# witalis3/UHSDR

Measured on AMD Instinct MI355X. Metric: Msamples/s through full SSB-RX chain (node); % of HBM-roofline per GPU, higher is better.
Workload: dtype f32; 1 GPU; C2: 4096 ch x 256-frame blocks, SSB-USB P48 chain, f32; channels_per_gpu=4096, frames_per_call=256, parallelism=channel-sharded x1, no data-path collective, outputs=f32 audio, pipelined=True, handoff=persistent, precision=exact, schedule=split_pipe

## Files before the change

### uhsdr_amd/csrc/uhsdr_dsp.h

```cpp
#ifndef UHSDR_DSP_H
#define UHSDR_DSP_H

#include <hip/hip_runtime.h>
#include <stdint.h>
#include "uhsdr_internal.h"

#define BLK UHSDR_IQ_BLOCK_SIZE
#define IQ_BIT_SCALE_DOWN 0.0000152587890625f

typedef float vf4 __attribute__((ext_vector_type(4)));

template <int V, int N>
__device__ __forceinline__ void lds_vec(const float* p, float (&w)[N], int j)
{
    if (V == 4)
    {
        const float4 v = *(const float4*)p;
        w[j] = v.x; w[j + 1] = v.y; w[j + 2] = v.z; w[j + 3] = v.w;
    }
    else
    {
        const float2 v = *(const float2*)p;
        w[j] = v.x; w[j + 1] = v.y;
    }
}

typedef const __attribute__((address_space(4))) float ctaps_t;
__device__ __forceinline__ ctaps_t* as_taps(const float* p) { return (ctaps_t*)p; }

template <bool F, typename V>
__device__ __forceinline__ V fir_mac(V acc, V x, V c)
{
    if constexpr (F) return __builtin_elementwise_fma(x, c, acc);
    else return acc + x * c;
}

template <int T, int R, int M, int V = 4, bool F = false, bool TP = false>
__device__ __forceinline__ void fir_block(const float* win, ctaps_t* c, float (&acc)[R])
{
    constexpr int WA = (M * (R - 1) + 8 + 7) & ~7;
    constexpr int NCH = T / 8, TR = T % 8;
    constexpr int ROT = NCH <= 8 ? (NCH > 0 ? NCH : 1) : WA / 8 + 1;
    float w[WA];
#pragma unroll
    for (int r = 0; r < R; ++r) acc[r] = 0.0f;
#pragma unroll
    for (int j = 0; j < WA; j += V) lds_vec<V>(win + j, w, j);
    float cn[8];
    if constexpr (TP)
    {
#pragma unroll
        for (int q = 0; q < 8; ++q) cn[q] = c[q];
    }
#pragma unroll ROT
    for (int ch = 0; ch < NCH; ++ch)
    {
        float cc[8];
        if constexpr (TP)
        {
#pragma unroll
            for (int q = 0; q < 8; ++q) cc[q] = cn[q];
#pragma unroll
            for (int q = 0; q < 8; ++q) cn[q] = c[8 * (ch + 1) + q];
        }
        else
        {
#pragma unroll
            for (int q = 0; q < 8; ++q) cc[q] = c[8 * ch + q];
        }
        float nw[8];
#pragma unroll
        for (int q = 0; q < 8; q += V) lds_vec<V>(win + 8 * ch + WA + q, nw, q);
#pragma unroll
        for (int kk = 0; kk < 8; ++kk)
        {
#pragma unroll
            for (int r = 0; r < R; ++r) acc[r] = fir_mac<F>(acc[r], w[r * M + kk], cc[kk]);
        }
#pragma unroll
        for (int j = 0; j < WA - 8; ++j) w[j] = w[j + 8];
#pragma unroll
        for (int q = 0; q < 8; ++q) w[WA - 8 + q] = nw[q];
    }
#pragma unroll
    for (int kk = 0; kk < TR; ++kk)
    {
        const float ck = TP ? cn[kk] : c[8 * NCH + kk];
#pragma unroll
        for (int r = 0; r < R; ++r) acc[r] = fir_mac<F>(acc[r], w[r * M + kk], ck);
    }
}

typedef float v2f __attribute__((ext_vector_type(2)));
typedef const __attribute__((address_space(4))) v2f ctaps2_t;
__device__ __forceinline__ ctaps2_t* as_taps2(const float* p) { return (ctaps2_t*)p; }

template <int PB>
__host__ __device__ constexpr int pwin_off(int i) { return 2 * i + PB * (i >> 3); }
__host__ __device__ constexpr int front_pad1(int R, bool decim_first, int M) { return R == 8 && (decim_first || M == 1) ? 4 : 0; }

template <int T, int R, int M, bool F = false, int PB = 0, bool TP = false>
__device__ __forceinline__ void fir_block2(const float* win, ctaps2_t* c, v2f (&acc)[R])
{
    constexpr int WA = (M * (R - 1) + 8 + 7) & ~7;
    constexpr int NCH = T / 8, TR = T % 8;
    constexpr int ROT = WA / 8 + 1;
    v2f w[WA];
#pragma unroll
    for (int r = 0; r < R; ++r) acc[r] = v2f{ 0.0f, 0.0f };
#pragma unroll
    for (int j = 0; j < WA; j += 2)
    {
        const vf4 v = *(const vf4*)(win + pwin_off<PB>(j));
        w[j] = v.xy; w[j + 1] = v.zw;
    }
    v2f cn[8];
    if constexpr (TP)
    {
#pragma unroll
        for (int q = 0; q < 8; ++q) cn[q] = c[q];
    }
#pragma unroll ROT
    for (int ch = 0; ch < NCH; ++ch)
    {
        v2f cc[8];
        if constexpr (TP)
        {
#pragma unroll
            for (int q = 0; q < 8; ++q) cc[q] = cn[q];
#pragma unroll
            for (int q = 0; q < 8; ++q) cn[q] = c[8 * (ch + 1) + q];
        }
        else
        {
#pragma unroll
            for (int q = 0; q < 8; ++q) cc[q] = c[8 * ch + q];
        }
        v2f nw[8];
#pragma unroll
        for (int q = 0; q < 8; q += 2)
        {
            const vf4 v = *(const vf4*)(win + (16 + PB) * ch + pwin_off<PB>(WA + q));
            nw[q] = v.xy; nw[q + 1] = v.zw;
        }
#pragma unroll
        for (int kk = 0; kk < 8; ++kk)
        {
#pragma unroll
            for (int r = 0; r < R; ++r) acc[r] = fir_mac<F>(acc[r], w[r * M + kk], cc[kk]);
        }
#pragma unroll
        for (int j = 0; j < WA - 8; ++j) w[j] = w[j + 8];
#pragma unroll
        for (int q = 0; q < 8; ++q) w[WA - 8 + q] = nw[q];
    }
#pragma unroll
    for (int kk = 0; kk < TR; ++kk)
    {
        const v2f ck = TP ? cn[kk] : c[8 * NCH + kk];
#pragma unroll
        for (int r = 0; r < R; ++r) acc[r] = fir_mac<F>(acc[r], w[r * M + kk], ck);
    }
}

constexpr int FRONT_TAIL = 8;

__device__ __forceinline__ float to_vgpr(float x)
{
    float r;
    asm volatile("v_mov_b32 %0, %1" : "=v"(r) : "s"(x));
    return r;
}
template <int N>
__device__ __forceinline__ void to_vgpr(float (&x)[N])
{
#pragma unroll
// ... 224 lines not shown
        const int q = lane + FRONT_WAVE_L * i;
        buf[i] = h[q < qmax ? q : qmax];
    }
}

template <int T, int PB = 0, int HQM>
__device__ __forceinline__ void group_fill_prow(float* smem, int LW, const float* row, int c0, int cpw, int nlive,
                                                int lane, const vf4 (&buf)[HQM])
{
    constexpr int hp4 = hist_p4(T), HQ = hist_qp(T);
    const int nq = cpw * hp4;
#pragma unroll
    for (int i = 0; i < HQ; ++i)
    {
        const int q = lane + FRONT_WAVE_L * i;
        if (q < nq) *(vf4*)(smem + (q / hp4) * LW + pwin_off<PB>(2 * (q % hp4))) = buf[i];
    }
    const vf4* h = (const vf4*)(row + (size_t)c0 * (hp4 * 4));
    const int qmax = nlive * hp4 - 1;
    for (int q = lane + FRONT_WAVE_L * HQ; q < nq; q += FRONT_WAVE_L)
        *(vf4*)(smem + (q / hp4) * LW + pwin_off<PB>(2 * (q % hp4))) = h[q < qmax ? q : qmax];
}

template <int T, int PB = 0>
__device__ __forceinline__ void group_store_prow(const float* smem, int LW, float* row, int c0, int nlive, int lane, int nnew)
{
    constexpr int hp4 = hist_p4(T);
    vf4* h = (vf4*)(row + (size_t)c0 * (hp4 * 4));
    for (int q = lane; q < nlive * hp4; q += FRONT_WAVE_L)
        h[q] = *(const vf4*)(smem + (q / hp4) * LW + pwin_off<PB>(nnew + 2 * (q % hp4)));
}

template <int PB = 0>
__device__ __forceinline__ void window_new2(float* W, int T, bool act, int b, const v2f* vals, int NV)
{
    if (act)
    {
        const int i0 = T - 1 + b * NV;
        if (((T - 1) & 1) == 0)
            for (int j = 0; j < NV; j += 2)
                *(vf4*)(W + pwin_off<PB>(i0 + j)) = vf4{ vals[j].x, vals[j].y, vals[j + 1].x, vals[j + 1].y };
        else
            for (int j = 0; j < NV; ++j) *(v2f*)(W + pwin_off<PB>(i0 + j)) = vals[j];
    }
}

__device__ __forceinline__ void window_new(float* W, int T, bool act, int b, const float* vals, int NV)
{
    if (act)
    {
        float* d = W + T - 1 + b * NV;
        if (((T - 1 + b * NV) & 3) == 0 && (NV & 3) == 0)
            for (int j = 0; j < NV; j += 4) *(vf4*)(d + j) = vf4{ vals[j], vals[j + 1], vals[j + 2], vals[j + 3] };
        else if (((T - 1 + b * NV) & 1) == 0 && (NV & 1) == 0)
            for (int j = 0; j < NV; j += 2) *(v2f*)(d + j) = v2f{ vals[j], vals[j + 1] };
        else
            for (int j = 0; j < NV; ++j) d[j] = vals[j];
    }
}

__host__ __device__ inline void front_lane(int l, int nb, int S, int& g, int& b)
{
    const int cpw = 64 / nb, K = 64 / S, cpg = S / 4;
    if ((nb & (nb - 1)) || nb < K || cpw < cpg)
    {
        g = l / nb;
        b = l % nb;
        return;
    }
    const int h = l & 31;
    int k, j;
    if (h < 4) { k = 0; j = h; }
    else if (h < 12) { k = 1; j = h - 4; }
    else if (h < 16) { k = 0; j = h - 8; }
    else if (h < 20) { k = 1; j = h - 8; }
    else if (h < 28) { k = 0; j = h - 12; }
    else { k = 1; j = h - 16; }
    k += (l >> 5) * 2;
    const int pr = k * cpg + j / K;
    g = pr % cpw;
    b = (pr / cpw) * K + j % K;
}

template <int S>
__device__ __forceinline__ float lattice_step(float x, float (&g)[S > 0 ? S : 1], const float* k, const float* v)
{
    float fcurr = x, fnext = 0.0f, acc = 0.0f;
    float gn[S > 0 ? S : 1];
#pragma unroll
    for (int i = 0; i < S; ++i)
    {
        const float gcurr = g[i];
        fnext = fcurr - (k[i] * gcurr);
        const float gnext = (fnext * k[i]) + gcurr;
        acc += (gnext * v[i]);
        gn[i] = gnext;
        fcurr = fnext;
    }
    acc += (fnext * v[S]);
#pragma unroll
    for (int i = 0; i + 1 < S; ++i) g[i] = gn[i + 1];
    if (S > 0) g[S - 1] = fnext;
    return acc;
}

template <int S, int PAR>
__device__ __forceinline__ float lattice_step_pk(float x, float (&g)[S > 0 ? S : 1], const float* k, const float* v)
{
    if constexpr (S < 3) return lattice_step<S>(x, g, k, v);
    else
    {
        float gn[S], q[S];
        float f = x;
        int i = 0;
        if (PAR)
        {
            f = f - (k[0] * g[0]);
            gn[0] = (f * k[0]) + g[0];
            q[0] = gn[0] * v[0];
            i = 1;
        }
#pragma unroll
        for (; i + 1 < S; i += 2)
        {
            const v2f gp = v2f{ g[i], g[i + 1] }, kp = v2f{ k[i], k[i + 1] };
            const v2f kg = kp * gp;
            const float f0 = f - kg.x;
            const float f1 = f0 - kg.y;
            const v2f gnp = (v2f{ f0, f1 } * kp) + gp;
            const v2f qp = gnp * v2f{ v[i], v[i + 1] };
            gn[i] = gnp.x; gn[i + 1] = gnp.y;
            q[i] = qp.x; q[i + 1] = qp.y;
            f = f1;
        }
        if (i < S)
        {
            f = f - (k[i] * g[i]);
            gn[i] = (f * k[i]) + g[i];
            q[i] = gn[i] * v[i];
        }
        float acc = 0.0f;
#pragma unroll
        for (int j = 0; j < S; ++j) acc += q[j];
        acc += (f * v[S]);
#pragma unroll
        for (int j = 0; j + 1 < S; ++j) g[j] = gn[j + 1];
        g[S - 1] = f;
        return acc;
    }
}

template <int S>
__device__ __forceinline__ void lattice_step2_pk(float x0, float x1, float (&g)[S > 0 ? S : 1], const float* k,
                                                 const float* v, float& y0, float& y1)
{
    static_assert(S >= 3, "packed form");
    float q[2][S + 1];
#pragma unroll
    for (int h = 0; h < 2; ++h)
    {
        float gn[S];
        float f = h ? x1 : x0;
        int i = 0;
        if (h)
        {
            f = f - (k[0] * g[0]);
            gn[0] = (f * k[0]) + g[0];
            q[h][0] = gn[0] * v[0];
            i = 1;
        }
#pragma unroll
        for (; i + 1 < S; i += 2)
        {
            const v2f gp = v2f{ g[i], g[i + 1] }, kp = v2f{ k[i], k[i + 1] };
            const v2f kg = kp * gp;
            const float f0 = f - kg.x;
            const float f1 = f0 - kg.y;
            const v2f gnp = (v2f{ f0, f1 } * kp) + gp;
            const v2f qp = gnp * v2f{ v[i], v[i + 1] };
            gn[i] = gnp.x; gn[i + 1] = gnp.y;
            q[h][i] = qp.x; q[h][i + 1] = qp.y;
            f = f1;
        }
        if (i < S)
        {
            f = f - (k[i] * g[i]);
            gn[i] = (f * k[i]) + g[i];
            q[h][i] = gn[i] * v[i];
        }
        q[h][S] = f * v[S];
#pragma unroll
        for (int j = 0; j + 1 < S; ++j) g[j] = gn[j + 1];
        g[S - 1] = f;
    }
    v2f acc = v2f{ 0.0f, 0.0f };
#pragma unroll
    for (int j = 0; j <= S; ++j) acc = acc + v2f{ q[0][j], q[1][j] };
    y0 = acc.x;
    y1 = acc.y;
}

__device__ __forceinline__ float biquad_step(float x, float& x1, float& x2, float& y1, float& y2, const float* c)
{
    const float acc = (c[0] * x) + (c[1] * x1) + (c[2] * x2) + (c[3] * y1) + (c[4] * y2);
    x2 = x1; x1 = x; y2 = y1; y1 = acc;
    return acc;
}

enum LdsOp { LDS_R128, LDS_W128, LDS_W64, LDS_W32 };
static const int kB128Groups[4][16] = {
    { 0, 1, 2, 3, 12, 13, 14, 15, 20, 21, 22, 23, 24, 25, 26, 27 },
    { 4, 5, 6, 7, 8, 9, 10, 11, 16, 17, 18, 19, 28, 29, 30, 31 },
    { 32, 33, 34, 35, 44, 45, 46, 47, 52, 53, 54, 55, 56, 57, 58, 59 },
    { 36, 37, 38, 39, 40, 41, 42, 43, 48, 49, 50, 51, 60, 61, 62, 63 } };

static inline int lds_op_cycles(LdsOp op, const int (&addr)[64])
{
    const int ngroups = op == LDS_R128 ? 4 : op == LDS_W128 ? 8 : op == LDS_W64 ? 4 : 2;
    const int glen = 64 / ngroups, banks = op == LDS_R128 ? 64 : 32;
    const int nd = op == LDS_W64 ? 2 : op == LDS_W32 ? 1 : 4;
    int cycles = 0;
    for (int gi = 0; gi < ngroups; ++gi)
    {
        int load[64] = { 0 }, seen[64], nseen = 0;
        for (int k = 0; k < glen; ++k)
        {
            const int l = op == LDS_R128 ? kB128Groups[gi][k] : gi * glen + k;
            if (addr[l] < 0) continue;
            for (int d = 0; d < nd; ++d)
            {
                const int ad = addr[l] + d;
                bool dup = false;
                for (int i = 0; i < nseen; ++i) dup = dup || seen[i] == ad;
                if (dup) continue;
                if (nseen < 64) seen[nseen++] = ad;
                load[ad & (banks - 1)] += 1;
            }
        }
        int mx = 0;
        for (int k = 0; k < 64; ++k) mx = load[k] > mx ? load[k] : mx;
        cycles += mx;
    }
    return cycles;
}

__host__ __device__ inline void front_lane(int l, int nb, int S, int& g, int& b);
static inline bool front_lane_interleaved(int l, int nb, int& g, int& b)
{
    if (nb > 16 || (nb & (nb - 1)) || 64 % (4 * nb)) return false;
    g = l % 4 + 4 * (l / (4 * nb));
    b = (l % (4 * nb)) / 4;
    return true;
}

static inline int front_lds_pass1(int lw, const uint16_t* lm, int cpw, int T1, int R, int pb = 0)
{
    auto off = [&](int i) { return 2 * i + pb * (i >> 3); };
    int addr[64], cycles = 0;
    for (int l = 0; l < 64; ++l)
    {
        const int g = lm[l] >> 8, b = lm[l] & 0xff;
        addr[l] = g < cpw ? g * lw + off(T1 - 1 + b * R) : -1;
    }
    cycles += lds_op_cycles(((T1 - 1) & 1) ? LDS_W64 : LDS_W128, addr) * (((T1 - 1) & 1) ? R : R / 2);
    const int WA = (R - 1 + 8 + 7) & ~7;
    for (int l = 0; l < 64; ++l)
    {
        const int g = lm[l] >> 8, b = lm[l] & 0xff;
        addr[l] = g < cpw ? g * lw + off(b * R) : -1;
    }
    return cycles + lds_op_cycles(LDS_R128, addr) * (WA / 2 + (T1 / 8) * 4);
}

static inline int front_lds_pass2(int lw, const uint16_t* lm1, const uint16_t* lm2, int cpw, int T2, bool pair2, int NV,
                                  int RD, int M2)
{
    int addr[64], cycles = 0;
    const int off = pair2 ? 2 * (T2 - 1) : T2 - 1, per = pair2 ? 2 * NV : NV;
    for (int l = 0; l < 64; ++l)
    {
        const int g = lm1[l] >> 8, b = lm1[l] & 0xff;
        addr[l] = g < cpw ? g * lw + off + b * per : -1;
    }
// ... 45 lines not shown
```

### uhsdr_amd/csrc/uhsdr_rx.hip

```cpp

#include <hip/hip_runtime.h>
#include <hip/hip_ext.h>
#include <stdint.h>
#include <string.h>
#include <stdlib.h>
#include <math.h>
#include <chrono>
#include "uhsdr_internal.h"
#include "uhsdr_libm.h"
#include "uhsdr_dsp.h"

#define BACK_CH 64
constexpr int CNT_PITCH = 32;

struct FrontArgs
{
    const uhsdr_rx_plan* plan;
    const int2* iq;
    float* hist1;
    float* hist2;
    const uint16_t* lanemap;
    const uint16_t* lanemap2;
    int nb, cpw;
    float* teta;
// ... 640 lines not shown
};


constexpr int CHAIN_ADP = BACK_CH + 4;

constexpr unsigned DFLAG_SPIN_MAX = 1u << 24;
__device__ __forceinline__ unsigned front_waves_of(const BackArgs& a, int g)
{
    const int c0 = g * BACK_CH, c1 = (c0 + BACK_CH < a.C ? c0 + BACK_CH : a.C) - 1;
    return (unsigned)(c1 / a.fcpw - c0 / a.fcpw + 1);
}
__device__ __forceinline__ void dflag_wait(const BackArgs& a, const unsigned* cnt, unsigned target, bool& gave_up)
{
    const int g = blockIdx.x;
    const unsigned want = target * front_waves_of(a, g);
    unsigned v = __hip_atomic_load(cnt + g * CNT_PITCH, __ATOMIC_RELAXED, __HIP_MEMORY_SCOPE_AGENT);
    for (unsigned spins = 0; (int)(v - want) < 0 && !gave_up; ++spins)
    {
        if (spins >= a.spin_max)
        {
            if ((threadIdx.x & (BACK_CH - 1)) == 0) __hip_atomic_store(a.fail, 1u, __ATOMIC_RELAXED, __HIP_MEMORY_SCOPE_SYSTEM);
            gave_up = true;
        }
        __builtin_amdgcn_s_sleep(2);
        v = __hip_atomic_load(cnt + g * CNT_PITCH, __ATOMIC_RELAXED, __HIP_MEMORY_SCOPE_AGENT);
    }
    __builtin_amdgcn_fence(__ATOMIC_ACQUIRE, "wavefront");
}

template <int L, bool LDS_IN = false, bool DW = false, bool PERS = false>
struct InStage
{
    static constexpr int NDC = BLK / L;
    float xnext[NDC];
    const float* lds;
    bool gave_up = false;
    int lim = -1;

    __device__ __forceinline__ void fetch(const BackArgs& a, const BackLane& l, int call)
    {
        if constexpr (LDS_IN)
        {
            const int col = l.cl - (l.c - l.lane);
#pragma unroll
            for (int m = 0; m < NDC; ++m) xnext[m] = lds[(call * NDC + m) * CHAIN_ADP + col];
            return;
        }
        if (DW && a.dwait)
        {
            if (call == 0) dflag_wait(a, a.dwait, a.dtarget, gave_up);
            if (PERS && a.pctl && call == l.calls) dflag_wait(a, a.dwait_next, a.dnext, gave_up);
            const float* src = call < l.calls ? a.adec + (size_t)l.cl * a.Nd + call * NDC
                                              : a.adec_next + (size_t)l.cl * a.Nd + (call - l.calls) * NDC;
#pragma unroll
            for (int m = 0; m < NDC; ++m)
            {
                const float v = __hip_atomic_load(src + m, __ATOMIC_RELAXED, __HIP_MEMORY_SCOPE_AGENT);
                xnext[m] = gave_up ? __builtin_nanf("") : v;
            }
            return;
        }
        const float* src = a.adec + call * NDC;
        const unsigned off = (unsigned)l.cl * (unsigned)a.Nd;
#pragma unroll
        for (int m = 0; m < NDC; m += 4)
        {
            const float4 v = *(const float4*)(src + m + off);
            xnext[m] = v.x; xnext[m + 1] = v.y; xnext[m + 2] = v.z; xnext[m + 3] = v.w;
        }
    }

    __device__ __forceinline__ void begin(const BackArgs& a, const BackLane& l, int call, float (&xin)[NDC])
    {
#pragma unroll
        for (int m = 0; m < NDC; ++m) xin[m] = xnext[m];
        if (call + 1 < (lim < 0 ? l.calls : lim)) fetch(a, l, call + 1);
    }
};

template <int S, bool PK = true>
struct LatticeStage
{
    float k[S > 0 ? S : 1], v[S + 1], g[S > 0 ? S : 1];

    __device__ __forceinline__ void load(const BackLane& l, const float* kc, const float* vc, const float* st)
    {
#pragma unroll
        for (int i = 0; i < S; ++i) k[i] = kc[i];
#pragma unroll
        for (int i = 0; i <= S; ++i) v[i] = vc[i];
#pragma unroll
        for (int i = 0; i < S; ++i) g[i] = st[i * l.C + l.cl];
    }

    __device__ __forceinline__ float step(float x, int par = 0)
    {
        if constexpr (S > 0 && PK) return (par & 1) ? lattice_step_pk<S, 1>(x, g, k, v) : lattice_step_pk<S, 0>(x, g, k, v);
        if constexpr (S > 0 && !PK) return lattice_step<S>(x, g, k, v);
        return x;
    }

    __device__ __forceinline__ void step2(float x0, float x1, float& y0, float& y1)
    {
        if constexpr (S >= 3 && PK) lattice_step2_pk<S>(x0, x1, g, k, v, y0, y1);
        else
        {
            y0 = step(x0, 0);
            y1 = step(x1, 1);
        }
    }

    __device__ __forceinline__ void store(const BackLane& l, float* st)
    {
        if (!l.live) return;
#pragma unroll
        for (int i = 0; i < S; ++i) st[i * l.C + l.c] = g[i];
    }
};

template <int L, int W, int NCH = 1>
struct AgcStage
{
    static constexpr int NDC = BLK / L;
    static_assert(W == AGC_Q * NDC + 1, "AGC window must be AGC_Q calls + 1 sample");
    bool agc_on, dc;
    bool dc_sel;
    float volts, save_volts, fast_bavg, hang_bavg, wold[NCH];
    float cmax[AGC_Q - 1];
    float leave_last[NCH];
    int hang_counter, decay_type, state;
    float rnext[NCH][NDC];
    float old[NCH][NDC], sfx[NDC], wmax, pmax;
    float* ring_out[NCH];
    int lim = -1;

    __device__ __forceinline__ static float* ring_of(const BackArgs& a, int ch) { return ch ? a.s.ring1 : a.s.ring; }

    __device__ __forceinline__ void load(const BackArgs& a, const BackLane& l, const uhsdr_agc_plan& A)
    {
        const int C = l.C, cl = l.cl;
        agc_on = A.mode != 5;
        dc = A.remove_dc != 0;
        dc_sel = false;
        volts = a.s.agc[1 * C + cl];
        save_volts = a.s.agc[2 * C + cl];
        fast_bavg = a.s.agc[3 * C + cl];
        hang_bavg = a.s.agc[4 * C + cl];
        wold[0] = a.s.agc[5 * C + cl];
#pragma unroll
        for (int i = 0; i < AGC_Q - 1; ++i) cmax[i] = a.s.agc[(6 + i) * C + cl];
        leave_last[0] = a.s.agc[(5 + AGC_Q) * C + cl];
        if (NCH == 2)
        {
            wold[NCH - 1] = a.s.agc[(6 + AGC_Q) * C + cl];
            leave_last[NCH - 1] = a.s.agc[(7 + AGC_Q) * C + cl];
        }
        hang_counter = a.s.agci[0 * C + cl];
        decay_type = a.s.agci[1 * C + cl];
        state = a.s.agci[2 * C + cl];
    }

    __device__ __forceinline__ void fetch(const BackArgs& a, const BackLane& l, int call)
    {
        if (agc_on)
        {
            const int slot = (a.ring_phase + call) % AGC_Q;
#pragma unroll
            for (int ch = 0; ch < NCH; ++ch)
            {
                const float* rs = ring_of(a, ch) + (size_t)slot * NDC * l.C;
#pragma unroll
                for (int m = 0; m < NDC; ++m) rnext[ch][m] = rs[(size_t)m * l.C + (unsigned)l.cl];
            }
        }
    }

    template <typename F>
    __device__ __forceinline__ static float absn(F&& v)
    {
        float r = fabsf(v(0));
#pragma unroll
        for (int ch = 1; ch < NCH; ++ch) r = fmaxf(r, fabsf(v(ch)));
        return r;
    }

    __device__ __forceinline__ void begin(const BackArgs& a, const BackLane& l, int call)
    {
#pragma unroll
        for (int ch = 0; ch < NCH; ++ch)
#pragma unroll
            for (int m = 0; m < NDC; ++m) old[ch][m] = rnext[ch][m];
// ... 1119 lines not shown
        br.template put<0, NDC>(l, lds.agc + o);
        br.template put<NDC, NDC>(l, lds.dem + o);
    }
    for (;;)
    {
    BACK_ROLE_LOOP(DM ? 3 : 2)
        const float* ai = lds.agc + (call & 1) * NDC * BACK_CH + l.lane;
        float* mo = lds.mid + (call & 1) * BLK * BACK_CH + l.lane;
        float x[NDC];
#pragma unroll
        for (int m = 0; m < NDC; ++m) x[m] = ai[m * BACK_CH];
        if (agc_on && (DM || (back_agc_split(DM) && !A.remove_dc)))
        {
            const float* vi = (DM ? lds.prep + 2 * NDC * BACK_CH : lds.dem) + (call & 1) * NDC * BACK_CH + l.lane;
            float v[NDC];
#pragma unroll
            for (int m = 0; m < NDC; ++m) v[m] = vi[m * BACK_CH];
#pragma unroll
            for (int m = 0; m < NDC; ++m) x[m] = x[m] * AgcStage<L, W, 1>::gain(v[m], A);
            if (dc)
            {
#pragma unroll
                for (int m = 0; m < NDC; ++m)
                {
                    const float w = (float)((double)x[m] + (double)wold * 0.9999);
                    x[m] = w - wold;
                    wold = w;
                }
            }
        }
#pragma unroll
        for (int m = 0; m < NDC; ++m)
        {
            float u[L];
            if constexpr (TAP)
            {
                const float t = s.step_dec(x[m]);
                if (l.live && call < l.calls) a.tap[(size_t)l.c * a.Nd + call * NDC + m] = t;
                s.interp(t, u);
            }
            else
                s.step(x[m], u);
#pragma unroll
            for (int j = 0; j < L; ++j) mo[(m * L + j) * BACK_CH] = u[j];
        }
        s.end(a, l, call);
    BACK_ROLE_END
        if (!pers || !back_ext(sch, lds)) break;
        sch = BackSched::next(l);
        glim = l.calls;
    }
    s.store(a, l);
    if (DM && l.live) a.s.agc[5 * l.C + l.c] = wold;
    if (back_ext(sch, lds))
    {
        const int o = ((l.calls + BACK_SKEW - 2) & 1) * NDC * BACK_CH;
        bnd_store<NDC>(a, l, 4 * NDC, lds.agc + o);
        bnd_store<NDC>(a, l, 5 * NDC, lds.dem + o);
    }
}

template <int AA, int DM, bool PERS>
__device__ __forceinline__ void rx_back_aa(const BackArgs& a, BackLds lds)
{
    const BackLane l(a);
    const uhsdr_rx_plan* __restrict__ P = a.plan;
    const int skw = BackSched::word<DM>(a);
    LatticeStage<AA> s;
    s.load(l, P->aa_k, P->aa_v, a.s.aa);
    BndRegs<BLK> br;
    br.template load<DM>(a, l, a.bnd_mid);
    BackSched sch = BackSched::make<DM, PERS>(a, l, skw);
    int glim = l.calls;
    const bool pers = PERS && DM == DM_NONE && a.pctl != nullptr;
    if (sch.pin) br.template put<0, BLK>(l, lds.mid + ((sch.gofs - 3) & 1) * BLK * BACK_CH);
    for (;;)
    {
    BACK_ROLE_LOOP(DM ? 4 : 3)
        const float* mi = lds.mid + (call & 1) * BLK * BACK_CH + l.lane;
        float* mo = lds.aa + (call & 1) * BLK * BACK_CH + l.lane;
        float x[BLK];
#pragma unroll
        for (int n = 0; n < BLK; ++n) x[n] = mi[n * BACK_CH];
#pragma unroll
        for (int n = 0; n < BLK; n += 2)
        {
            float y0, y1;
            s.step2(x[n], x[n + 1], y0, y1);
            mo[n * BACK_CH] = y0;
            mo[(n + 1) * BACK_CH] = y1;
        }
    BACK_ROLE_END
        if (!pers || !back_ext(sch, lds)) break;
        sch = BackSched::next(l);
        glim = l.calls;
    }
    s.store(l, a.s.aa);
    if (back_ext(sch, lds)) bnd_store<BLK>(a, l, a.bnd_mid, lds.mid + ((l.calls + BACK_SKEW - 3) & 1) * BLK * BACK_CH);
}

constexpr int BACK_TAILS = 4;
__host__ __device__ constexpr int back_tails(int dm) { return dm == DM_NONE ? BACK_TAILS : 0; }
template <int DM, bool PERS>
__device__ __forceinline__ void rx_back_output(const BackArgs& a, BackLds lds)
{
    const BackLane l(a);
    const int skw = BackSched::word<DM>(a);
    OutputStage s;
    s.load(a, l);
    BndRegs<BLK> br;
    br.template load<DM>(a, l, a.bnd_mid + BLK);
    BackSched sch = BackSched::make<DM, PERS>(a, l, skw);
    int glim = l.calls;
    const bool pers = PERS && DM == DM_NONE && a.pctl != nullptr;
    if (sch.pin) br.template put<0, BLK>(l, lds.aa + ((sch.gofs - 4) & 1) * BLK * BACK_CH);
    bool pread = !sch.pin;
    for (;;)
    {
    BACK_ROLE_LOOP(DM ? 5 : 4)
        const float* mi = lds.aa + (call & 1) * BLK * BACK_CH + l.lane;
        float y[BLK];
#pragma unroll
        for (int n = 0; n < BLK; ++n) y[n] = mi[n * BACK_CH];
#pragma unroll
        for (int n = 0; n < BLK; ++n) y[n] = s.step(y[n]);
        if constexpr (DM == DM_NONE)
        {
            if (pread && a.dwait && __builtin_amdgcn_readfirstlane(*lds.poison))
            {
#pragma unroll
                for (int n = 0; n < BLK; ++n) y[n] = __builtin_nanf("");
            }
        }
        float* yl = lds.ys + (call & 1) * BACK_CH * FUSED_YPITCH + l.lane * FUSED_YPITCH;
#pragma unroll
        for (int n = 0; n < BLK; ++n) yl[n] = y[n];
        if constexpr (back_tails(DM) == 0) fused_store_call(a, l, call, lds.ys + (call & 1) * BACK_CH * FUSED_YPITCH);
    BACK_ROLE_END
        if (!pers || !back_ext(sch, lds)) break;
        sch = BackSched::next(l);
        glim = l.calls;
        pread = true;
    }
    s.store(a, l);
    if (back_ext(sch, lds)) bnd_store<BLK>(a, l, a.bnd_mid + BLK, lds.aa + ((l.calls + BACK_SKEW - 4) & 1) * BLK * BACK_CH);
}
#undef BACK_ROLE_LOOP

template <int DM, bool PERS>
__device__ __forceinline__ void rx_back_tail(const BackArgs& a0, BackLds lds, int half)
{
    BackArgs a = a0;
    const BackLane l(a);
    BackSched sch = BackSched::make<DM, PERS>(a, l, BackSched::word<DM>(a));
    const bool pers = PERS && DM == DM_NONE && a.pctl != nullptr;
    constexpr int ST = back_roles(DM);
    const int g8 = l.lane >> 3, j = l.lane & 7;
    const int c0 = l.c - l.lane;
    auto store_call = [&](int call) {
        const float* ys = lds.ys + (call & 1) * BACK_CH * FUSED_YPITCH;
        constexpr int KT = 8 / (back_tails(DM) ? back_tails(DM) : 1);
#pragma unroll
        for (int kk = 0; kk < KT; ++kk)
        {
            const int k = half * KT + kk;
            const int cc = 8 * k + g8;
            const float* r = ys + cc * FUSED_YPITCH + 4 * j;
            const float v[4] = { r[0], r[1], r[2], r[3] };
            if (c0 + cc >= a.C) continue;
            const size_t rb = (size_t)(c0 + 8 * k) * a.N + call * BLK;
            const unsigned off = (unsigned)g8 * (unsigned)a.N + 4 * j;
            line_out4(a, rb, off, call, call * BLK + 4 * j, v);
        }
    };
// ... 726 lines not shown
constexpr int TAPS2_MAX = (UHSDR_MAX_FIR_TAPS + 7) & ~7;
constexpr int BACK_FUSED_MIN_CHANNELS = 131072;

constexpr int PIPE_GROUP = 4;
constexpr int PIPE_BUFS = 2 * PIPE_GROUP;

struct uhsdr_rx_s
{
    uhsdr_rx_plan plan;
    uhsdr_rx_plan* d_plan;
    const FrontVariant* fv;
    const BackVariant* bv;
    const NotchVariant* nv;
    const ChainVariant* cv;
    int C, N, Nd, Nf;
    int lw;
    int schedule;
    int precision;
    int T1, T2;
    hipStream_t stream;
    float *hist1, *hist2, *teta, *osc, *adec, *adec_q;
    uint16_t* d_lanemap;
    uint16_t lmap[2][2][64];
    int* tp;
    unsigned* clip;
    float* d_taps2;
    BackState bs;
    void* arena;
    size_t arena_bytes;
    long long dec_samples;
    int cw_count;
    int cw_bmax, cw_blocks_last;
    int beep_left;
    uint32_t beep_acc;
    uint8_t* cw_signal;
    float* cw_energy;
    uhsdr_cwdec_handle cwt;
    uint8_t* cwt_signal;
    float* tap;
    uhsdr_rtty_handle rtty;
    uhsdr_psk_handle psk;
    float* text_tap;
    long long calls_done;
    long long front_launches;
    int pipelined;
    hipStream_t side;
    hipEvent_t ev_front, ev_join, ev_back[2];
    hipEvent_t ev_switch;
    float *adecp[PIPE_BUFS - 1], *adec_qp[PIPE_BUFS - 1];
    long long calls_issued;
    long long pipe_calls;
    int side_dirty;
    struct
    {
        int timing;
        int tsample;
        long long tcalls;
        int nev;
        int nev_cap;
        hipEvent_t* ev;
        uint8_t* evmask;
        float total_ms[4];
        int launches[4];
    } tim;
    volatile unsigned* fail_host;
    unsigned* fail_dev;
    unsigned spin_max;
    struct
    {
        int dflag;
        unsigned* gcnt;
        unsigned fills[PIPE_BUFS];
        int* skew;
        float* bnd;
        int dflag_grid;
        int back_attr;
    } hand;
    int pers;
    struct
    {
        unsigned* pmem;
        unsigned* pmem_dev;
        unsigned* pdec;
        int plive, pprev;
        unsigned plast;
        unsigned pepoch;
    } run;
    int main_back;
};

enum { K_FRONT = 0, K_BACK = 1, K_CHAIN = 2, NKERN = 3 };
static const char* kKernelNames[NKERN] = { "rx_front", "rx_back", "rx_chain" };

static bool side_mode(const uhsdr_rx_s* h) { return h->pipelined; }
static hipStream_t back_stream(const uhsdr_rx_s* h) { return side_mode(h) ? h->side : h->stream; }

static void time_mark(uhsdr_rx_s* h, int k, int which)
{
    if (!h->tim.tsample) return;
    (void)hipEventRecord(h->tim.ev[((size_t)h->tim.nev * NKERN + k) * 2 + which], k == K_BACK ? back_stream(h) : h->stream);
    if (which) h->tim.evmask[h->tim.nev] |= (uint8_t)(1u << k);
}

static void pers_close(uhsdr_rx_s* h)
{
    h->run.plive = 0;
}

static hipError_t sync_all(uhsdr_rx_s* h)
{
    pers_close(h);
    hipError_t e = hipStreamSynchronize(h->stream);
    if (e == hipSuccess && h->side) e = hipStreamSynchronize(h->side);
    return e;
}

static void time_harvest(uhsdr_rx_s* h)
{
    if (!h->tim.nev) return;
    (void)sync_all(h);
    for (int i = 0; i < h->tim.nev; ++i)
        for (int k = 0; k < NKERN; ++k)
        {
            float ms = 0.0f;
            const size_t e = ((size_t)i * NKERN + k) * 2;
            if ((h->tim.evmask[i] >> k & 1) && hipEventElapsedTime(&ms, h->tim.ev[e], h->tim.ev[e + 1]) == hipSuccess)
            {
                h->tim.total_ms[k] += ms;
                h->tim.launches[k] += 1;
            }
        }
    h->tim.nev = 0;
}

#define HIPCHK(x) do { hipError_t e_ = (x); if (e_ != hipSuccess) { uhsdr_set_error("%s: %s", #x, hipGetErrorString(e_)); return UHSDR_DEVICE_ERROR; } } while (0)

static size_t front_lds_extra(const uhsdr_rx_s* h);
constexpr size_t LDS_PER_CU = 160 * 1024;

static int kernel_waves_per_cu(const void* fn)
{
    hipFuncAttributes at;
    if (hipFuncGetAttributes(&at, fn) != hipSuccess || at.numRegs <= 0) return 16;
    const int alloc = (at.numRegs + 7) & ~7;
    const int w = 512 / alloc;
    return 4 * (w > 8 ? 8 : w);
}
constexpr int FRONT_SLACK = 2 * FRONT_TAIL;

static int front_window_pitch(const uhsdr_rx_s* h, uint16_t (&lm1_out)[64], uint16_t (&lm2_out)[64])
{
    const int N = h->Nf, R = h->fv->R, M = h->plan.decimation_rate;
    const bool df = h->plan.use_decimated_iq;
    const bool pair2 = df || h->fv->st;
    const int nb = N / R, cpw = FRONT_WAVE / nb;
    const int n2 = df ? N / M : N;
    const int pb1 = front_pad1(R, h->fv->decim_first != 0, h->fv->m);
    int need = pb1 ? pwin_off<4>(h->T1 - 1 + N + FRONT_TAIL) : 2 * (h->T1 - 1 + N);
    const int need2 = h->T2 ? (pair2 ? 2 : 1) * (h->T2 - 1 + n2) : 0;
    need = ((need > need2 ? need : need2) + 3) & ~3;
    const int RD = R / M;
    const int NV2 = df ? RD : R, RD2 = df ? RD : RD, M2 = df ? 1 : M;
    const int S2 = (pair2 ? 2 : 1) * NV2;
    const size_t extra = front_lds_extra(h) + FRONT_SLACK;
    const int vgpr_waves = kernel_waves_per_cu((const void*)h->fv->fn);
    uint16_t maps[3][64];
    int nmaps = 0;
// ... 696 lines not shown
{
    if (!*h->fail_host) return UHSDR_OK;
    uhsdr_set_error("the pipelined device hand-off gave up waiting for rx_front (a poll bound of %u polls): the "
                    "outputs of that call are poisoned (NaN audio) and the handle's state is invalid until "
                    "uhsdr_rx_reset", h->spin_max);
    return UHSDR_TIMEOUT;
}


#define RXSTEP(x) do { const uhsdr_status s_ = (x); if (s_ != UHSDR_OK) return s_; } while (0)

static uhsdr_status chain_call(uhsdr_rx_s* h, const int32_t* iq, float* audio, float* audio0, int32_t* dst, bool fma)
{
    if (side_mode(h) && h->side_dirty)
    {
        HIPCHK(hipEventRecord(h->ev_join, h->side));
        HIPCHK(hipStreamWaitEvent(h->stream, h->ev_join, 0));
        h->side_dirty = 0;
    }
    const FrontArgs fa = front_args(h, iq, 0, nullptr, nullptr);
    const BackArgs ba = back_args(h, nullptr, nullptr, audio, audio0, dst);
    time_mark(h, K_CHAIN, 0);
    const chain_fn cfn = ba.tap ? (fma ? h->cv->fn_tap_fma : h->cv->fn_tap) : fma ? h->cv->fn_fma : h->cv->fn;
    hipLaunchKernelGGL(cfn, dim3((h->C + BACK_CH - 1) / BACK_CH), dim3(FRONT_WAVE),
                       chain_lds(h), h->stream, fa, ba, (int)chain_front_floats(h));
    HIPCHK(hipGetLastError());
    time_mark(h, K_CHAIN, 1);
    h->main_back = 1;
    h->front_launches += 1;
    return UHSDR_OK;
}

struct RxRoute
{
    long long pk;
    int par;
    int grp;
    bool group_end;
    float *adec, *adec_q;
    int cpw;
    int bgroups;
    unsigned* gc;
    bool side;
    bool fused;
    bool dfl;
    bool pm;
    unsigned seq;
};

static RxRoute route_call(const uhsdr_rx_s* h)
{
    RxRoute r;
    r.pk = h->pipe_calls;
    r.par = h->pipelined ? (int)(r.pk % PIPE_BUFS) : 0;
    r.grp = (int)((r.pk / PIPE_GROUP) & 1);
    r.group_end = h->pipelined && r.pk % PIPE_GROUP == PIPE_GROUP - 1;
    r.adec = r.par ? h->adecp[r.par - 1] : h->adec;
    r.adec_q = r.par ? h->adec_qp[r.par - 1] : h->adec_q;
    r.cpw = FRONT_WAVE / (h->Nf / h->fv->R);
    r.side = side_mode(h);
    r.fused = h->schedule == UHSDR_SCHEDULE_SPLIT_FUSED || h->plan.stereo;
    r.bgroups = (h->C + BACK_CH - 1) / BACK_CH;
    r.dfl = r.side && h->hand.dflag && !h->main_back && !r.fused && !h->nv && !h->fv->st &&
            h->bv->dm == DM_NONE && r.bgroups <= h->hand.dflag_grid;
    r.gc = h->hand.gcnt + (size_t)r.par * r.bgroups * CNT_PITCH;
    r.pm = r.dfl && h->pers && h->hand.skew && h->N / BLK >= 2 * BACK_SKEW && !h->bs.cw && !tap_row(h) &&
           r.bgroups <= PC_MAX_GROUPS && h->bv->fn_pers;
    r.seq = (unsigned)r.pk;
    return r;
}

static uhsdr_status pers_begin(uhsdr_rx_s* h, const RxRoute& r)
{
    unsigned* const pw = h->run.pmem;
    if (!r.pm && h->run.plive) HIPCHK(sync_all(h));
    if (r.pm && !h->run.pprev)
    {
        HIPCHK(sync_all(h));
        HIPCHK(hipMemsetAsync(h->run.pdec, 0xFF, sizeof(unsigned) * DESC_RING * PDEC_PITCH, h->side));
        for (int g = 0; g < r.bgroups; ++g) __atomic_store_n(pw + PC_CONSUMED + g, r.seq, __ATOMIC_SEQ_CST);
        __atomic_store_n(pw + PC_GRANT, 0u, __ATOMIC_SEQ_CST);
        __atomic_store_n(pw + PC_EXIT, r.seq - 2, __ATOMIC_SEQ_CST);
        __atomic_store_n(pw + PC_DECIDED, ((r.seq - 2) << 1) | 1u, __ATOMIC_SEQ_CST);
    }
    h->run.pprev = r.pm;
    return UHSDR_OK;
}

template <class Pred>
static uhsdr_status pers_spin(Pred done, const char* what, unsigned call)
{
    if (done()) return UHSDR_OK;
    const auto t0 = std::chrono::steady_clock::now();
    for (;;)
    {
        if (std::chrono::steady_clock::now() - t0 > std::chrono::seconds(30))
        {
            uhsdr_set_error(what, call);
            return UHSDR_TIMEOUT;
        }
        if (done()) return UHSDR_OK;
    }
}

static uhsdr_status wait_release(uhsdr_rx_s* h, const RxRoute& r)
{
    if (r.pm)
    {
        const unsigned* pw = h->run.pmem;
        const unsigned need = r.seq - (PIPE_BUFS - 1);
        return pers_spin([&]() {
            for (int g = 0; g < r.bgroups; ++g)
                if ((int)(__atomic_load_n(pw + PC_CONSUMED + g, __ATOMIC_ACQUIRE) - need) < 0) return false;
            return true;
        }, "persistent back end: call %u's hand-off buffer not released within 30 s", r.seq);
    }
    if (r.side && r.pk % PIPE_GROUP == 0) HIPCHK(hipStreamWaitEvent(h->stream, h->ev_back[r.grp], 0));
    return UHSDR_OK;
}

static uhsdr_status launch_fronts(uhsdr_rx_s* h, const RxRoute& r, const int32_t* iq, bool fma)
{
    const size_t lds = front_lds(h);
    time_mark(h, K_FRONT, 0);
    for (int f0 = 0; f0 < h->N; f0 += h->Nf)
    {
        FrontArgs fa = front_args(h, iq, f0, r.adec, r.adec_q);
        if (r.dfl)
        {
            fa.gcnt = r.gc;
            h->hand.fills[r.par] += 1;
        }
        const auto fn = fma ? h->fv->fn_fma : h->fv->fn;
        const dim3 grid((h->C + r.cpw - 1) / r.cpw), block(FRONT_WAVE);
        if (r.side && !r.dfl && f0 + h->Nf >= h->N)
            hipExtLaunchKernelGGL(fn, grid, block, lds, h->stream, nullptr, h->ev_front, 0, fa);
        else
            hipLaunchKernelGGL(fn, grid, block, lds, h->stream, fa);
        HIPCHK(hipGetLastError());
        h->front_launches += 1;
    }
    time_mark(h, K_FRONT, 1);
    return UHSDR_OK;
}

static void handoff_args(const uhsdr_rx_s* h, const RxRoute& r, BackArgs& bk)
{
    bk.dwait = r.gc;
    bk.dtarget = h->hand.fills[r.par];
    bk.fcpw = r.cpw;
    if (h->hand.skew && h->N / BLK >= BACK_SKEW && !h->bs.cw && !bk.tap)
    {
        const int parn = (int)((r.pk + 1) % PIPE_BUFS);
        bk.adec_next = parn ? h->adecp[parn - 1] : h->adec;
        bk.dwait_next = h->hand.gcnt + (size_t)parn * r.bgroups * CNT_PITCH;
        bk.dnext = h->hand.fills[parn] + (unsigned)((h->N + h->Nf - 1) / h->Nf);
    }
}

static uhsdr_status pers_grant(uhsdr_rx_s* h, const RxRoute& r, BackArgs& bk, bool& launch)
{
    unsigned* const pw = h->run.pmem;
    const unsigned seq = r.seq;
    BackDesc* d = (BackDesc*)(pw + PC_WORDS) + seq % DESC_RING;
    d->adec = r.adec;
    d->cnt = r.gc;
    d->audio = bk.audio;
    d->audio0 = bk.audio0;
    d->dst = bk.dst;
    d->target = h->hand.fills[r.par];
    d->beep_n0 = bk.beep_n0;
    d->beep_n1 = bk.beep_n1;
    d->beep_acc = bk.beep_acc;
    __atomic_store_n(&d->seq, seq, __ATOMIC_RELEASE);
    auto grant = [&]() { return h->run.pepoch << 24 | (seq & 0xFFFFFFu); };
    launch = true;
    if (h->run.plive)
    {
        __atomic_store_n(pw + PC_GRANT, grant(), __ATOMIC_SEQ_CST);
        launch = false;
        if (__atomic_load_n(pw + PC_EXIT, __ATOMIC_SEQ_CST) == seq - 1)
        {
            const unsigned want = (seq - 1) & 0x7FFFFFFFu;
            unsigned dv = 0;
            RXSTEP(pers_spin([&]() { return ((dv = __atomic_load_n(pw + PC_DECIDED, __ATOMIC_ACQUIRE)) >> 1) == want; },
                             "persistent back end: no decision after call %u within 30 s", seq - 1));
            launch = dv & 1u;
        }
    }
    h->run.plast = seq;
    if (launch)
    {
        h->run.pepoch = (h->run.pepoch + 1) & 0xFFu;
        __atomic_store_n(pw + PC_GRANT, grant(), __ATOMIC_SEQ_CST);
        bk.pepoch = h->run.pepoch;
        bk.pctl = h->run.pmem_dev;
        bk.pdesc = (const BackDesc*)(h->run.pmem_dev + PC_WORDS);
        bk.pdec = h->run.pdec;
        bk.seq0 = seq;
        bk.adec_next = nullptr;
        bk.dwait_next = nullptr;
        h->run.plive = 1;
    }
    return UHSDR_OK;
}

static size_t back_launch_lds(uhsdr_rx_s* h, const RxRoute& r)
{
    if (r.fused) return 0;
    if (r.dfl)
    {
        if (!h->hand.back_attr)
        {
            h->hand.back_attr = hipFuncSetAttribute((const void*)h->bv->fn, hipFuncAttributeMaxDynamicSharedMemorySize,
                                                    (int)LDS_PER_CU) == hipSuccess ? 1 : -1;
            if (h->hand.back_attr > 0 && h->bv->fn_pers &&
                hipFuncSetAttribute((const void*)h->bv->fn_pers, hipFuncAttributeMaxDynamicSharedMemorySize,
                                    (int)LDS_PER_CU) != hipSuccess)
                h->hand.back_attr = -1;
            if (h->hand.back_attr > 0 && h->bv->fn_tap &&
                hipFuncSetAttribute((const void*)h->bv->fn_tap, hipFuncAttributeMaxDynamicSharedMemorySize,
                                    (int)LDS_PER_CU) != hipSuccess)
                h->hand.back_attr = -1;
            (void)hipGetLastError();
        }
        if (h->hand.back_attr > 0) return LDS_PER_CU - 4096;
    }
    return back_lds(h);
}

static uhsdr_status launch_back(uhsdr_rx_s* h, const RxRoute& r, const BackArgs& bk, bool launch)
{
    const hipStream_t bst = back_stream(h);
    if (r.side && !r.dfl) HIPCHK(hipStreamWaitEvent(bst, h->ev_front, 0));
    time_mark(h, K_BACK, 0);
    if (h->nv)
    {
        hipLaunchKernelGGL(h->nv->fn, dim3((h->C + BACK_CH - 1) / BACK_CH), dim3(BACK_CH), 0, bst, bk);
        HIPCHK(hipGetLastError());
    }
    const back_fn bfn = r.fused ? (bk.tap ? h->bv->fused_tap : fused_back_fn(h)) : r.pm ? h->bv->fn_pers : bk.tap ? h->bv->fn_tap : h->bv->fn;
    const int bwaves = r.fused ? 1 : h->bv->dm == DM_FM ? back_roles(DM_FM) : back_roles(h->bv->dm) + back_tails(h->bv->dm);
    const dim3 bgrid((h->C + BACK_CH - 1) / BACK_CH), bblock(bwaves * BACK_CH);
    const size_t blds = back_launch_lds(h, r);
    if (r.pm)
    {
        if (launch) hipLaunchKernelGGL(bfn, bgrid, bblock, blds, bst, bk);
    }
    else if (r.side && r.group_end)
        hipExtLaunchKernelGGL(bfn, bgrid, bblock, blds, bst, nullptr, h->ev_back[r.grp], 0, bk);
    else
        hipLaunchKernelGGL(bfn, bgrid, bblock, blds, bst, bk);
    HIPCHK(hipGetLastError());
    time_mark(h, K_BACK, 1);
    return UHSDR_OK;
}

static uhsdr_status rx_process(uhsdr_rx_handle h, const int32_t* iq, float* audio, float* audio0, int32_t* dst)
{
    if (!h || !iq) { uhsdr_set_error("null argument"); return UHSDR_ARGUMENT_ERROR; }
    RXSTEP(check_fail(h));
    if (h->tim.timing && h->tim.nev >= h->tim.nev_cap) time_harvest(h);
    h->tim.tsample = h->tim.timing && (h->tim.tcalls++ % h->tim.timing) == 0;
    if (h->tim.tsample) h->tim.evmask[h->tim.nev] = 0;
    const bool fma = h->precision == UHSDR_PRECISION_FMA;
    const int cw0 = h->cw_count;
    if (h->schedule == UHSDR_SCHEDULE_CHAIN)
    {
        RXSTEP(chain_call(h, iq, audio, audio0, dst, fma));
        RXSTEP(launch_cw_text(h, cw0, h->stream));
        RXSTEP(launch_rtty_text(h, h->stream));
        RXSTEP(launch_psk_text(h, h->stream));
    }
    else
    {
// ... 310 lines not shown
```

Measured before the change: 57140 Msamples/s.

## Skew lattice filter across sample pairs to pack stages into v2f ops

Moves the lattice helpers into their own header and adds a software-pipelined whole-block lattice runner. It processes an even and an odd sample offset by half the stage count, so each step does two stages at once with packed v2f multiply-adds. Stage coefficient pairs are precomputed at load time, and the back end now runs the lattice over the whole block instead of sample pairs. Separately, the host now waits for the previous persistent launch to report closed before relaunching, which adds a possible host spin. The skewed schedule raises register pressure from the per-step R/F arrays.

Measured after the change: 54210 Msamples/s. -5.1%, worse.

```diff
diff --git a/uhsdr_amd/csrc/uhsdr_dsp.h b/uhsdr_amd/csrc/uhsdr_dsp.h
--- a/uhsdr_amd/csrc/uhsdr_dsp.h
+++ b/uhsdr_amd/csrc/uhsdr_dsp.h
@@ -4,6 +4,7 @@
 #include <hip/hip_runtime.h>
 #include <stdint.h>
 #include "uhsdr_internal.h"
+#include "uhsdr_lattice.h"
 
 #define BLK UHSDR_IQ_BLOCK_SIZE
 #define IQ_BIT_SCALE_DOWN 0.0000152587890625f
@@ -91,7 +92,6 @@
     }
 }
 
-typedef float v2f __attribute__((ext_vector_type(2)));
 typedef const __attribute__((address_space(4))) v2f ctaps2_t;
 __device__ __forceinline__ ctaps2_t* as_taps2(const float* p) { return (ctaps2_t*)p; }
 
@@ -482,123 +482,6 @@
     b = (pr / cpw) * K + j % K;
 }
 
-template <int S>
-__device__ __forceinline__ float lattice_step(float x, float (&g)[S > 0 ? S : 1], const float* k, const float* v)
-{
-    float fcurr = x, fnext = 0.0f, acc = 0.0f;
-    float gn[S > 0 ? S : 1];
-#pragma unroll
-    for (int i = 0; i < S; ++i)
-    {
-        const float gcurr = g[i];
-        fnext = fcurr - (k[i] * gcurr);
-        const float gnext = (fnext * k[i]) + gcurr;
-        acc += (gnext * v[i]);
-        gn[i] = gnext;
-        fcurr = fnext;
-    }
-    acc += (fnext * v[S]);
-#pragma unroll
-    for (int i = 0; i + 1 < S; ++i) g[i] = gn[i + 1];
-    if (S > 0) g[S - 1] = fnext;
-    return acc;
-}
-
-template <int S, int PAR>
-__device__ __forceinline__ float lattice_step_pk(float x, float (&g)[S > 0 ? S : 1], const float* k, const float* v)
-{
-    if constexpr (S < 3) return lattice_step<S>(x, g, k, v);
-    else
-    {
-        float gn[S], q[S];
-        float f = x;
-        int i = 0;
-        if (PAR)
-        {
-            f = f - (k[0] * g[0]);
-            gn[0] = (f * k[0]) + g[0];
-            q[0] = gn[0] * v[0];
-            i = 1;
-        }
-#pragma unroll
-        for (; i + 1 < S; i += 2)
-        {
-            const v2f gp = v2f{ g[i], g[i + 1] }, kp = v2f{ k[i], k[i + 1] };
-            const v2f kg = kp * gp;
-            const float f0 = f - kg.x;
-            const float f1 = f0 - kg.y;
-            const v2f gnp = (v2f{ f0, f1 } * kp) + gp;
-            const v2f qp = gnp * v2f{ v[i], v[i + 1] };
-            gn[i] = gnp.x; gn[i + 1] = gnp.y;
-            q[i] = qp.x; q[i + 1] = qp.y;
-            f = f1;
-        }
-        if (i < S)
-        {
-            f = f - (k[i] * g[i]);
-            gn[i] = (f * k[i]) + g[i];
-            q[i] = gn[i] * v[i];
-        }
-        float acc = 0.0f;
-#pragma unroll
-        for (int j = 0; j < S; ++j) acc += q[j];
-        acc += (f * v[S]);
-#pragma unroll
-        for (int j = 0; j + 1 < S; ++j) g[j] = gn[j + 1];
-        g[S - 1] = f;
-        return acc;
-    }
-}
-
-template <int S>
-__device__ __forceinline__ void lattice_step2_pk(float x0, float x1, float (&g)[S > 0 ? S : 1], const float* k,
-                                                 const float* v, float& y0, float& y1)
-{
-    static_assert(S >= 3, "packed form");
-    float q[2][S + 1];
-#pragma unroll
-    for (int h = 0; h < 2; ++h)
-    {
-        float gn[S];
-        float f = h ? x1 : x0;
-        int i = 0;
-        if (h)
-        {
-            f = f - (k[0] * g[0]);
-            gn[0] = (f * k[0]) + g[0];
-            q[h][0] = gn[0] * v[0];
-            i = 1;
-        }
-#pragma unroll
-        for (; i + 1 < S; i += 2)
-        {
-            const v2f gp = v2f{ g[i], g[i + 1] }, kp = v2f{ k[i], k[i + 1] };
-            const v2f kg = kp * gp;
-            const float f0 = f - kg.x;
-            const float f1 = f0 - kg.y;
-            const v2f gnp = (v2f{ f0, f1 } * kp) + gp;
-            const v2f qp = gnp * v2f{ v[i], v[i + 1] };
-            gn[i] = gnp.x; gn[i + 1] = gnp.y;
-            q[h][i] = qp.x; q[h][i + 1] = qp.y;
-            f = f1;
-        }
-        if (i < S)
-        {
-            f = f - (k[i] * g[i]);
-            gn[i] = (f * k[i]) + g[i];
-            q[h][i] = gn[i] * v[i];
-        }
-        q[h][S] = f * v[S];
-#pragma unroll
-        for (int j = 0; j + 1 < S; ++j) g[j] = gn[j + 1];
-        g[S - 1] = f;
-    }
-    v2f acc = v2f{ 0.0f, 0.0f };
-#pragma unroll
-    for (int j = 0; j <= S; ++j) acc = acc + v2f{ q[0][j], q[1][j] };
-    y0 = acc.x;
-    y1 = acc.y;
-}
 
 __device__ __forceinline__ float biquad_step(float x, float& x1, float& x2, float& y1, float& y2, const float* c)
 {
diff --git a/uhsdr_amd/csrc/uhsdr_lattice.h b/uhsdr_amd/csrc/uhsdr_lattice.h
--- /dev/null
+++ b/uhsdr_amd/csrc/uhsdr_lattice.h
@@ -0,0 +1,225 @@
+#ifndef UHSDR_LATTICE_H
+#define UHSDR_LATTICE_H
+
+#include <utility>
+
+typedef float v2f __attribute__((ext_vector_type(2)));
+
+template <int S>
+__device__ __forceinline__ float lattice_step(float x, float (&g)[S > 0 ? S : 1], const float* k, const float* v)
+{
+    float fcurr = x, fnext = 0.0f, acc = 0.0f;
+    float gn[S > 0 ? S : 1];
+#pragma unroll
+    for (int i = 0; i < S; ++i)
+    {
+        const float gcurr = g[i];
+        fnext = fcurr - (k[i] * gcurr);
+        const float gnext = (fnext * k[i]) + gcurr;
+        acc += (gnext * v[i]);
+        gn[i] = gnext;
+        fcurr = fnext;
+    }
+    acc += (fnext * v[S]);
+#pragma unroll
+    for (int i = 0; i + 1 < S; ++i) g[i] = gn[i + 1];
+    if (S > 0) g[S - 1] = fnext;
+    return acc;
+}
+
+template <int S, int PAR>
+__device__ __forceinline__ float lattice_step_pk(float x, float (&g)[S > 0 ? S : 1], const float* k, const float* v)
+{
+    if constexpr (S < 3) return lattice_step<S>(x, g, k, v);
+    else
+    {
+        float gn[S], q[S];
+        float f = x;
+        int i = 0;
+        if (PAR)
+        {
+            f = f - (k[0] * g[0]);
+            gn[0] = (f * k[0]) + g[0];
+            q[0] = gn[0] * v[0];
+            i = 1;
+        }
+#pragma unroll
+        for (; i + 1 < S; i += 2)
+        {
+            const v2f gp = v2f{ g[i], g[i + 1] }, kp = v2f{ k[i], k[i + 1] };
+            const v2f kg = kp * gp;
+            const float f0 = f - kg.x;
+            const float f1 = f0 - kg.y;
+            const v2f gnp = (v2f{ f0, f1 } * kp) + gp;
+            const v2f qp = gnp * v2f{ v[i], v[i + 1] };
+            gn[i] = gnp.x; gn[i + 1] = gnp.y;
+            q[i] = qp.x; q[i + 1] = qp.y;
+            f = f1;
+        }
+        if (i < S)
+        {
+            f = f - (k[i] * g[i]);
+            gn[i] = (f * k[i]) + g[i];
+            q[i] = gn[i] * v[i];
+        }
+        float acc = 0.0f;
+#pragma unroll
+        for (int j = 0; j < S; ++j) acc += q[j];
+        acc += (f * v[S]);
+#pragma unroll
+        for (int j = 0; j + 1 < S; ++j) g[j] = gn[j + 1];
+        g[S - 1] = f;
+        return acc;
+    }
+}
+
+template <int S>
+__device__ __forceinline__ void lattice_step2_pk(float x0, float x1, float (&g)[S > 0 ? S : 1], const float* k,
+                                                 const float* v, float& y0, float& y1)
+{
+    static_assert(S >= 3, "packed form");
+    float q[2][S + 1];
+#pragma unroll
+    for (int h = 0; h < 2; ++h)
+    {
+        float gn[S];
+        float f = h ? x1 : x0;
+        int i = 0;
+        if (h)
+        {
+            f = f - (k[0] * g[0]);
+            gn[0] = (f * k[0]) + g[0];
+            q[h][0] = gn[0] * v[0];
+            i = 1;
+        }
+#pragma unroll
+        for (; i + 1 < S; i += 2)
+        {
+            const v2f gp = v2f{ g[i], g[i + 1] }, kp = v2f{ k[i], k[i + 1] };
+            const v2f kg = kp * gp;
+            const float f0 = f - kg.x;
+            const float f1 = f0 - kg.y;
+            const v2f gnp = (v2f{ f0, f1 } * kp) + gp;
+            const v2f qp = gnp * v2f{ v[i], v[i + 1] };
+            gn[i] = gnp.x; gn[i + 1] = gnp.y;
+            q[h][i] = qp.x; q[h][i + 1] = qp.y;
+            f = f1;
+        }
+        if (i < S)
+        {
+            f = f - (k[i] * g[i]);
+            gn[i] = (f * k[i]) + g[i];
+            q[h][i] = gn[i] * v[i];
+        }
+        q[h][S] = f * v[S];
+#pragma unroll
+        for (int j = 0; j + 1 < S; ++j) g[j] = gn[j + 1];
+        g[S - 1] = f;
+    }
+    v2f acc = v2f{ 0.0f, 0.0f };
+#pragma unroll
+    for (int j = 0; j <= S; ++j) acc = acc + v2f{ q[0][j], q[1][j] };
+    y0 = acc.x;
+    y1 = acc.y;
+}
+
+template <int S, int N, int T_>
+__device__ __forceinline__ void lattice_run_step(const float* x, const float* g, const float* k, const float* v,
+                                                 const v2f* kp2, const v2f* vp2, float* y, v2f* R, v2f* F, v2f& acc)
+{
+    constexpr int D = S / 2, M = N / 2, t = T_;
+    constexpr int i = t % S, j = (t + D) % S;
+    constexpr int ma = t / S, mb = t >= D ? (t - D) / S : 0;
+    constexpr bool A = t < M * S, B = t >= D;
+    constexpr int tr = t >= D - 1 ? t - D + 1 : 0, tf = t >= D ? t - D : 0, tp = t >= 1 ? t - 1 : 0;
+    float ga = 0.0f, gb = 0.0f, fa = 0.0f, fb = 0.0f;
+    if constexpr (A)
+    {
+        ga = ma == 0 ? g[i] : i < S - 1 ? R[tr].y : F[tf].y;
+        fa = i == 0 ? x[2 * ma] : F[tp].x;
+    }
+    if constexpr (B)
+    {
+        gb = j < S - 1 ? R[tr].x : F[tf].x;
+        fb = j == 0 ? x[2 * mb + 1] : F[tp].y;
+    }
+    v2f f = v2f{ fa, fb }, gn = v2f{ 0.0f, 0.0f };
+    if constexpr (A && B)
+    {
+        const v2f kp = i < D ? kp2[i] : __builtin_shufflevector(kp2[j], kp2[j], 1, 0);
+        const v2f vp = i < D ? vp2[i] : __builtin_shufflevector(vp2[j], vp2[j], 1, 0);
+        const v2f gp = v2f{ ga, gb };
+        f = f - (kp * gp);
+        gn = (f * kp) + gp;
+        const v2f q = gn * vp;
+        acc = v2f{ i == 0 ? 0.0f : acc.x, j == 0 ? 0.0f : acc.y } + q;
+    }
+    else if constexpr (A)
+    {
+        f.x = fa - (k[i] * ga);
+        gn.x = (f.x * k[i]) + ga;
+        acc.x = (i == 0 ? 0.0f : acc.x) + (gn.x * v[i]);
+    }
+    else
+    {
+        f.y = fb - (k[j] * gb);
+        gn.y = (f.y * k[j]) + gb;
+        acc.y = (j == 0 ? 0.0f : acc.y) + (gn.y * v[j]);
+    }
+    F[t] = f;
+    R[t] = gn;
+    if constexpr (A && i == S - 1) y[2 * ma] = acc.x + (f.x * v[S]);
+    if constexpr (B && j == S - 1) y[2 * mb + 1] = acc.y + (f.y * v[S]);
+}
+
+template <int S, int N, int... Ts>
+__device__ __forceinline__ void lattice_run_steps(std::integer_sequence<int, Ts...>, const float* x, const float* g,
+                                                  const float* k, const float* v, const v2f* kp2, const v2f* vp2, float* y,
+                                                  v2f* R, v2f* F, v2f& acc)
+{
+    (lattice_run_step<S, N, Ts>(x, g, k, v, kp2, vp2, y, R, F, acc), ...);
+}
+
+template <int S>
+__device__ __forceinline__ void lattice_pairs(const float* k, const float* v, v2f* kp2, v2f* vp2)
+{
+#pragma unroll
+    for (int i = 0; i < S / 2; ++i)
+    {
+        kp2[i] = v2f{ k[i], k[i + S / 2] };
+        vp2[i] = v2f{ v[i], v[i + S / 2] };
+    }
+}
+
+template <int S, int N>
+__device__ __forceinline__ void lattice_run_pk(const float (&x)[N > 0 ? N : 1], float (&g)[S > 0 ? S : 1], const float* k,
+                                               const float* v, const v2f* kp2, const v2f* vp2, float (&y)[N > 0 ? N : 1])
+{
+    if constexpr (S < 4 || (S & 1) || N < 2)
+    {
+#pragma unroll
+        for (int n = 0; n < N; ++n) y[n] = (n & 1) ? lattice_step_pk<S, 1>(x[n], g, k, v) : lattice_step_pk<S, 0>(x[n], g, k, v);
+    }
+    else
+    {
+        constexpr int M = N / 2, T = M * S + S / 2;
+        v2f R[T], F[T];
+        v2f acc = v2f{ 0.0f, 0.0f };
+        lattice_run_steps<S, N>(std::make_integer_sequence<int, T>{}, x, g, k, v, kp2, vp2, y, R, F, acc);
+#pragma unroll
+        for (int i = 0; i + 1 < S; ++i) g[i] = R[T - S + i + 1].y;
+        g[S - 1] = F[T - 1].y;
+        if constexpr (N & 1) y[N - 1] = lattice_step_pk<S, 0>(x[N - 1], g, k, v);
+    }
+}
+
+template <int S, int N>
+__device__ __forceinline__ void lattice_run_pk(const float (&x)[N > 0 ? N : 1], float (&g)[S > 0 ? S : 1], const float* k,
+                                               const float* v, float (&y)[N > 0 ? N : 1])
+{
+    v2f kp2[S > 1 ? S / 2 : 1], vp2[S > 1 ? S / 2 : 1];
+    lattice_pairs<S>(k, v, kp2, vp2);
+    lattice_run_pk<S, N>(x, g, k, v, kp2, vp2, y);
+}
+
+#endif
diff --git a/uhsdr_amd/csrc/uhsdr_rx.hip b/uhsdr_amd/csrc/uhsdr_rx.hip
--- a/uhsdr_amd/csrc/uhsdr_rx.hip
+++ b/uhsdr_amd/csrc/uhsdr_rx.hip
@@ -746,6 +746,7 @@
 struct LatticeStage
 {
     float k[S > 0 ? S : 1], v[S + 1], g[S > 0 ? S : 1];
+    v2f kp2[S > 1 ? S / 2 : 1], vp2[S > 1 ? S / 2 : 1];
 
     __device__ __forceinline__ void load(const BackLane& l, const float* kc, const float* vc, const float* st)
     {
@@ -753,6 +754,7 @@
         for (int i = 0; i < S; ++i) k[i] = kc[i];
 #pragma unroll
         for (int i = 0; i <= S; ++i) v[i] = vc[i];
+        if constexpr (S > 0 && PK) lattice_pairs<S>(kc, vc, kp2, vp2);
 #pragma unroll
         for (int i = 0; i < S; ++i) g[i] = st[i * l.C + l.cl];
     }
@@ -764,13 +766,14 @@
         return x;
     }
 
-    __device__ __forceinline__ void step2(float x0, float x1, float& y0, float& y1)
-    {
-        if constexpr (S >= 3 && PK) lattice_step2_pk<S>(x0, x1, g, k, v, y0, y1);
+    template <int N>
+    __device__ __forceinline__ void run(const float (&x)[N], float (&y)[N])
+    {
+        if constexpr (S > 0 && PK) lattice_run_pk<S, N>(x, g, k, v, kp2, vp2, y);
         else
         {
-            y0 = step(x0, 0);
-            y1 = step(x1, 1);
+#pragma unroll
+            for (int n = 0; n < N; ++n) y[n] = step(x[n], n);
         }
     }
 
@@ -2056,14 +2059,10 @@
         float x[BLK];
 #pragma unroll
         for (int n = 0; n < BLK; ++n) x[n] = mi[n * BACK_CH];
-#pragma unroll
-        for (int n = 0; n < BLK; n += 2)
-        {
-            float y0, y1;
-            s.step2(x[n], x[n + 1], y0, y1);
-            mo[n * BACK_CH] = y0;
-            mo[(n + 1) * BACK_CH] = y1;
-        }
+        float y[BLK];
+        s.template run<BLK>(x, y);
+#pragma unroll
+        for (int n = 0; n < BLK; ++n) mo[n * BACK_CH] = y[n];
     BACK_ROLE_END
         if (!pers || !back_ext(sch, lds)) break;
         sch = BackSched::next(l);
@@ -2956,7 +2955,7 @@
         unsigned* pmem;
         unsigned* pmem_dev;
         unsigned* pdec;
-        int plive, pprev;
+        int plive, pprev, pfresh;
         unsigned plast;
         unsigned pepoch;
     } run;
@@ -3819,6 +3818,7 @@
         __atomic_store_n(pw + PC_GRANT, 0u, __ATOMIC_SEQ_CST);
         __atomic_store_n(pw + PC_EXIT, r.seq - 2, __ATOMIC_SEQ_CST);
         __atomic_store_n(pw + PC_DECIDED, ((r.seq - 2) << 1) | 1u, __ATOMIC_SEQ_CST);
+        h->run.pfresh = 1;
     }
     h->run.pprev = r.pm;
     return UHSDR_OK;
@@ -3928,6 +3928,13 @@
     h->run.plast = seq;
     if (launch)
     {
+        if (!h->run.pfresh)
+        {
+            const unsigned closed = ((seq - 1) << 1) | 1u;
+            RXSTEP(pers_spin([&]() { return __atomic_load_n(pw + PC_DECIDED, __ATOMIC_ACQUIRE) == closed; },
+                             "persistent back end: the launch before call %u did not close within 30 s", seq));
+        }
+        h->run.pfresh = 0;
         h->run.pepoch = (h->run.pepoch + 1) & 0xFFu;
         __atomic_store_n(pw + PC_GRANT, grant(), __ATOMIC_SEQ_CST);
         bk.pepoch = h->run.pepoch;
```
